# junipertcy/bipartiteSBM-MCMC

Hardware: AMD Instinct MI355X
Metric: node-label MH updates/s (higher is better)
Workload: dtype f64

## Files before the change

### bipartitesbm-mcmc_amd/build.py

```python
import os
import shutil
import subprocess
import sys

HERE = os.path.dirname(os.path.abspath(__file__))
CSRC = os.path.join(HERE, "csrc")
LIB = os.path.join(HERE, "libbisbm_hip.so")
SOURCES = ["bisbm_kernels.hip", "bisbm_sweep_fast.hip", "bisbm_handle.hip", "bisbm_anneal.hip", "bisbm_marginals.hip",
           "bisbm_multi.hip", "bisbm_merge.hip", "bisbm_align.hip", "bisbm_tempering.hip", "bisbm_population.hip", "bisbm_pair_scores.hip", "bisbm_partition.hip",
           "bisbm_query_scores.hip", "bisbm_coassign.hip", "bisbm_foldin.hip", "bisbm_topk.hip", "bisbm_conditionals.hip", "bisbm_heatbath.hip", "bisbm_reshuffle.hip",
           "bisbm_mode_marginals.hip", "bisbm_trace.hip", "bisbm_block_sums.hip", "bisbm_clamp.hip",
           "bisbm_tables.cpp", "bisbm_io.cpp"]
HEADERS = ["bisbm_device.hpp", "bisbm_partition_device.hpp", "bisbm_kernels.hpp", "bisbm_stand_rule.hpp", "bisbm_move_word.hpp", "bisbm_predict_skew.hpp", "bisbm_engine.hpp", "bisbm_pass_policy.hpp", "bisbm_wave_chain.hpp", "bisbm_cand_lanes.hpp", os.path.join("..", "host", "bisbm.hpp"),
           os.path.join("..", "host", "mcmc_main.cpp"), os.path.join("..", "..", "include", "bisbm.h"),
           os.path.join("..", "..", "include", "bisbm_io.h")]
FLAGS = ["--offload-arch=gfx950", "-O3", "-std=c++17", "-ffp-contract=off", "-fPIC", "-pthread",
         "-Wall", "-Wno-unused-function",
         "-mllvm", "-structurizecfg-skip-uniform-regions=true",
         "-mllvm", "-amdgpu-atomic-optimizer-strategy=None",
         "-falign-loops=64"]


def hipcc():
    for cand in (shutil.which("hipcc"), "/opt/rocm/bin/hipcc"):
        if cand and os.path.exists(cand):
            return cand
    raise RuntimeError("hipcc not found: the engine is HIP-only and cannot be built without ROCm")


def needs_build():
    if not os.path.exists(LIB):
        return True
    t = os.path.getmtime(LIB)
    deps = [os.path.join(CSRC, s) for s in SOURCES + HEADERS] + [os.path.abspath(__file__)]
    return any(os.path.getmtime(d) > t for d in deps)


def build(force=False, verbose=False):
    import fcntl
    if not force and not needs_build():
        return LIB
    with open(os.path.join(HERE, ".build.lock"), "w") as lock:
        fcntl.flock(lock, fcntl.LOCK_EX)
        try:
            if not force and not needs_build():
                return LIB
            return _build_locked(verbose)
        finally:
            fcntl.flock(lock, fcntl.LOCK_UN)


RESOURCES = os.path.join(HERE, "libbisbm_hip.resources.json")


def _resource_usage(remarks):
    import re
    out, cur = {}, None
    for line in remarks.splitlines():
        m = re.search(r"remark:\s+Function Name: (\S+)", line)
        if m:
            cur = out.setdefault(m.group(1), {})
            continue
        m = re.search(r"remark:\s+([A-Za-z][^:]*): (\S+) \[-Rpass-analysis", line)
        if m and cur is not None:
            v = m.group(2)
            cur[m.group(1).strip()] = int(v) if v.isdigit() else v
    return out


def compile_library(out, extra=(), verbose=False, jobs=None):
    import tempfile
    from concurrent.futures import ThreadPoolExecutor
    cc = hipcc()
    objdir = tempfile.mkdtemp(prefix="bisbm_obj_")
    try:
        units = []
        for src in SOURCES:
            if src == "bisbm_sweep_fast.hip" and not any("BISBM_STAMPS" in f or "BISBM_PASS_COUNTS" in f for f in extra):
                units += [(src, ["-DBISBM_FAST_PART=%d" % part], "%s.part%d.o" % (src, part)) for part in range(5)]
            else:
                units.append((src, [], src + ".o"))

        def one(unit):
            src, defs, objname = unit
            obj = os.path.join(objdir, objname)
            cmd = [cc] + FLAGS + ["-Rpass-analysis=kernel-resource-usage"] + list(extra) + defs + ["-c", "-o", obj, os.path.join(CSRC, src)]
            if verbose:
                print(" ".join(cmd), file=sys.stderr)
            r = subprocess.run(cmd, capture_output=True, text=True)
            if r.returncode != 0:
                raise RuntimeError("hipcc failed on %s:\n%s%s" % (src, r.stdout, r.stderr))
            return obj, r.stderr
        with ThreadPoolExecutor(max_workers=jobs or min(len(units), os.cpu_count() or 1)) as pool:
            done = list(pool.map(one, units))
        tmp = out + ".tmp%d" % os.getpid()
        cmd = [cc, "--offload-arch=gfx950", "-shared", "-fPIC", "-pthread", "-o", tmp] + [o for o, _ in done]
# ... 50 lines not shown
```

### bipartitesbm-mcmc_amd/csrc/bisbm_sweep_fast.hip

```cpp
#include "bisbm_kernels.hpp"
#include "bisbm_move_word.hpp"
#include "bisbm_stand_rule.hpp"

#include <algorithm>
#include <cstdio>
#include <type_traits>

namespace bisbm {

#ifdef BISBM_STAMPS
__device__ unsigned long long g_fast_stamps[16];
#define FSTAMP(i)                                                                        \
    do {                                                                                 \
        unsigned long long now_;                                                         \
        __builtin_amdgcn_sched_barrier(0);                                               \
        __asm__ volatile("s_memtime %0\n\ts_waitcnt lgkmcnt(0)" : "=s"(now_)::"memory"); \
        __builtin_amdgcn_sched_barrier(0);                                               \
        st_acc[i] += now_ - st_prev;                                                     \
        st_prev = now_;                                                                  \
    } while (0)
#else
#define FSTAMP(i) \
    do {          \
    } while (0)
#endif
#if defined(BISBM_STAMPS) && BISBM_STAMPS == 2
#define FSTAMP_STEP(i) \
    do {               \
    } while (0)
#else
#define FSTAMP_STEP(i) FSTAMP(i)
#endif

__device__ __forceinline__ void wfence() {
    __builtin_amdgcn_wave_barrier();
    __asm__ volatile("" ::: "memory");
}

__device__ __forceinline__ double tab_at(const double* base, uint32_t idx) {
#if defined(BISBM_ABLATE) && (BISBM_ABLATE & 8)
    return (double)idx * 1e-3 + (double)((size_t)base & 0xff);
#endif
    return *(const double*)((const char*)base + (uint32_t)(idx << 3));
}

struct __attribute__((packed, aligned(4))) Id4 {
    uint32_t x, y, z, w;
};

__device__ __forceinline__ uint32_t sflag(uint32_t x) {
    uint32_t r;
    __asm__("s_min_u32 %0, %1, 1" : "=s"(r) : "s"(x) : "scc");
    return r;
}
__device__ __forceinline__ uint32_t smin(uint32_t x, uint32_t y) {
    uint32_t r;
    __asm__("s_min_u32 %0, %1, %2" : "=s"(r) : "s"(x), "s"(y) : "scc");
    return r;
}

struct LaneSwaps {
    __device__ __forceinline__ void swap16(int a, int b, int& x, int& y) const {
        const auto r = __builtin_amdgcn_permlane16_swap(a, b, false, false);
        x = (int)r[0], y = (int)r[1];
    }
    __device__ __forceinline__ void swap32(int a, int b, int& x, int& y) const {
        const auto r = __builtin_amdgcn_permlane32_swap(a, b, false, false);
        x = (int)r[0], y = (int)r[1];
    }
};


#ifdef BISBM_PASS_COUNTS
constexpr int kPassCounts = 15;
__device__ unsigned long long g_pass_counts[kPassCounts];
#define PCOUNT(i, v) (pc_acc[i] += (v))
#define PASS_COUNTS_PAIR(paired)                                                          \
    do {                                                                                  \
        const uint32_t pm_ = (paired) & chA, colk_ = col & sflag(kAtB) & (set_clash ^ 1u); \
        const uint32_t mv_ = target_moves(margin, kAtB);                                  \
        pc_acc[0] += 1u;                                                                  \
        pc_acc[1] += 1u + stands;                                                         \
        pc_acc[2] += pm_;                                                                 \
        pc_acc[3] += pm_ & set_clash;                                                     \
        pc_acc[4] += pm_ & colk_ & (mv_ ^ 1u);                                            \
        pc_acc[5] += pm_ & colk_ & mv_;                                                   \
        pc_acc[6] += pm_ & colk_ & (margin == kAtB ? 1u : 0u);                            \
        pc_acc[7] += pm_ & colk_ & (margin + 1u == kAtB ? 1u : 0u);                       \
    } while (0)
#else
#define PCOUNT(i, v) \
    do {             \
    } while (0)
#define PASS_COUNTS_PAIR(paired) \
    do {                         \
    } while (0)
#endif

#ifndef BISBM_PREDICT_TARGET
#define BISBM_PREDICT_TARGET 1
#endif
constexpr uint32_t kHistStride = 68;
constexpr uint32_t kHandWords = 9;
constexpr uint32_t kRowCap = 255;

#define BISBM_PIN(name, value) \
    double name = (value);     \
    __asm__ volatile("" : "+v"(name))

struct TargetReads {
    uint32_t s_loc, a_st, e_idx, tail_idx;
    int32_t m_st_raw, m_st;
    int ee, qn, qk;
    double logn, tail_lg, L2, L4;
};
struct TargetReads2 {
    uint32_t s_loc, a_st0, a_st1, e_idx, tail_idx;
    int32_t m_st_raw0, m_st_raw1, m_st0, m_st1;
    int ee, qn, qk;
    double logn, tail_lg, L2_0, L2_1, L4_0, L4_1;
};

struct PairSteps {
    uint32_t r_locA, r_locB, degA, degB, t_locB, s_prdA, s_prdB;
    uint32_t liveA, liveB;
    uint32_t selfA, selfB, warmA, warmB;
    uint32_t prop, pack_v, deg, r_loc, t_loc;
    double u_acc;
    __device__ __forceinline__ uint32_t flags(uint32_t clash) const {
        return (liveA & (selfA ^ 1u)) | ((liveA & selfA & warmA) << 1) | ((liveB & (selfB ^ 1u)) << 2) | ((liveB & selfB & warmB) << 3) |
               (clash << 4);
    }
};

__device__ __forceinline__ uint32_t rows4(unsigned long long b) {
    const unsigned long long x = b >> 15;
    return (uint32_t)(x | (x >> 15) | (x >> 30) | (x >> 45)) & 0xfu;
}
__device__ __forceinline__ void commit_four(uint32_t nst, uint32_t clash_bits, uint32_t mv4, uint32_t& moved, uint32_t& commit) {
    const uint32_t c01 = (clash_bits >> 1) & 1u, c02 = (clash_bits >> 2) & 1u, c03 = (clash_bits >> 3) & 1u;
    const uint32_t c12 = (clash_bits >> 6) & 1u, c13 = (clash_bits >> 7) & 1u, c23 = (clash_bits >> 11) & 1u;
    const uint32_t m0 = mv4 & 1u;
    const uint32_t k1 = sflag(nst - 1u) & ((m0 & c01) ^ 1u);
    const uint32_t m1 = k1 & (mv4 >> 1) & 1u;
    const uint32_t k2 = k1 & (nst > 2u ? 1u : 0u) & ((m0 & c02) ^ 1u) & ((m1 & c12) ^ 1u);
    const uint32_t m2 = k2 & (mv4 >> 2) & 1u;
    const uint32_t k3 = k2 & (nst > 3u ? 1u : 0u) & ((m0 & c03) ^ 1u) & ((m1 & c13) ^ 1u) & ((m2 & c23) ^ 1u);
    const uint32_t m3 = k3 & (mv4 >> 3) & 1u;
    commit = 1u | (k1 << 1) | (k2 << 2) | (k3 << 3);
    moved = m0 | (m1 << 1) | (m2 << 2) | (m3 << 3);
}

template <bool EL, bool CT, bool K32, bool K16, bool K8, bool Q32, bool OS>
__device__ __forceinline__ void sweep_fast_body(const SweepParams& p) {
    extern __shared__ __align__(16) uint32_t lds32[];
    const uint32_t chain = blockIdx.x;
    if (chain >= p.n_chains) return;
    const uint32_t lane = threadIdx.x & 63u;
    if (p.resume != 0u && p.scalars[chain].stopped != 0u) {
        if (threadIdx.x == 0) {
            p.scalars[chain].last_accepted = 0;
            p.scalars[chain].last_sweeps = 0;
        }
        return;
    }
    const uint32_t ka = p.ka, kb = p.kb, K = ka + kb, na = p.na, nb = p.nb;
    const uint32_t D = p.maxdeg + 1, S = kb | 1u;
    constexpr bool kPredictTarget = !K16 && (!Q32 || OS) && (BISBM_PREDICT_TARGET != 0);
    const uint32_t row_cap = p.maxdeg < kRowCap ? p.maxdeg : kRowCap;
    const uint32_t o_mq = 0, o_eta = ka * S;
    const uint32_t eta_w = EL ? D : p.eta_w;
    const uint32_t o_hist8 = o_eta + (EL ? K * D : (ka > kb ? ka : kb) * eta_w);
    const uint32_t o_hand = o_hist8 + 2 * kWave * (kHistStride / 4);
    const uint32_t o_slow = o_hand + 2 * kHandWords * kWave;
    const uint32_t o_flag = o_slow + kWave;
    int32_t* const mq = (int32_t*)(lds32 + o_mq);
    uint32_t* const eta_l = lds32 + o_eta;
    uint32_t* const hist8_base = lds32 + o_hist8;
    uint32_t* const hand_base = lds32 + o_hand;
    int32_t* const slow_hist = (int32_t*)(lds32 + o_slow);
    uint32_t* const stop_flag = lds32 + o_flag;
    unsigned long long* const below1_total = (unsigned long long*)(lds32 + ((o_flag + 4u + 1u) & ~1u));
    const uint32_t wave_in_wg = (uint32_t)__builtin_amdgcn_readfirstlane((int)(threadIdx.x >> 6));
    uint32_t hw_id, xcc_id;
    __asm__ volatile("s_getreg_b32 %0, hwreg(HW_REG_HW_ID)" : "=s"(hw_id));
    __asm__ volatile("s_getreg_b32 %0, hwreg(HW_REG_XCC_ID)" : "=s"(xcc_id));
    uint32_t* const role = lds32 + o_flag + 1;
    uint8_t* const new_lab = (uint8_t*)(lds32 + o_flag + 8);
    int32_t* const mr_pub = (int32_t*)(lds32 + o_flag + 24);
    double* const invT_buf = (double*)(lds32 + o_flag + 88);
    if (lane == 0) role[wave_in_wg] = ((xcc_id & 0xfu) << 10) | ((hw_id >> 6) & 0x3fcu) | ((hw_id >> 4) & 3u);
    __syncthreads();
    if (wave_in_wg == 0 && lane == 0) {
        uint32_t pick = p.simd_claims != nullptr ? 0u : (p.fixed_stepping_wave & 1u);
        if (p.simd_claims != nullptr && atomicAdd(&p.simd_claims[role[0]], 1u) != 0u) {
            if (atomicAdd(&p.simd_claims[role[1]], 1u) == 0u) {
                pick = 1;
                atomicSub(&p.simd_claims[role[0]], 1u);
            } else {
                atomicSub(&p.simd_claims[role[1]], 1u);
            }
        }
        role[2] = pick;
    }
    __syncthreads();
    const bool is_main = (uint32_t)__builtin_amdgcn_readfirstlane((int)role[2]) == wave_in_wg;

    uint8_t* const labels = p.labels + (size_t)chain * p.label_stride;
    int32_t* const m_g = p.m + (size_t)chain * ka * kb;
    int32_t* const mr_g = p.m_r + (size_t)chain * K;
    int32_t* const nr_g = p.n_r + (size_t)chain * K;
    uint32_t* const eta_g = p.eta + (size_t)chain * K * D;
    ChainScalars* const sc = p.scalars + chain;
    const Tables tab{p.lgamma_tab, p.lgamma_size, p.q_tab, p.q_stride, p.log_tab};
    if (lane == 0) {
        sc->hw_id[is_main ? 0 : 1] = hw_id;
        if (is_main) sc->xcc_id = xcc_id;
    }

    if (is_main) {
        for (uint32_t i = lane; i < ka * kb; i += kWave) mq[(i / kb) * S + (i % kb)] = m_g[i];
        if (EL)
            for (uint32_t i = lane; i < K * D; i += kWave) eta_l[i] = eta_g[i];
        if (lane == 0) {
            *stop_flag = 0;
            *below1_total = p.resume != 0u ? sc->stop_below1 : 0ull;
        }
    }
    if (is_main) __builtin_amdgcn_s_setprio(3);
    const uint32_t lb = K8 ? (lane & 7u) : K16 ? (lane & 15u) : K32 ? (lane & 31u) : lane;
    int mrA = lb < ka ? mr_g[lb] : 0, nrA = lb < ka ? nr_g[lb] : 0;
    int mrB = lb < kb ? mr_g[ka + lb] : 0, nrB = lb < kb ? nr_g[ka + lb] : 0;
    __syncthreads();
    uint64_t sweeps_total = sc->sweeps_total;

    const double eps = p.epsilon;
    const double Kd = (double)K;
    const double epsK = eps * Kd;
    const uint32_t chain_gid = chain_gid_of(p, chain);
    const uint32_t n = p.n;
    const uint64_t all_sweeps = p.duration / n;
    const double T_const = (double)p.kw0;
    const bool pair_mode = (uint32_t)__builtin_amdgcn_readfirstlane((K32 && (!CT || T_const > 0.) && p.pair_steps != 0) ? 1 : 0) != 0u;
    const bool pair64_mode = (uint32_t)__builtin_amdgcn_readfirstlane((!K32 && (!CT || T_const > 0.) && p.pair_steps != 0) ? 1 : 0) != 0u;
    const bool quad_mode = (uint32_t)__builtin_amdgcn_readfirstlane((K16 && !K8 && (!CT || T_const > 0.) && p.pair_steps > 1u) ? 1 : 0) != 0u;
    const bool quad32_mode = (uint32_t)__builtin_amdgcn_readfirstlane((Q32 && (!CT || T_const > 0.) && p.pair_steps > 1u) ? 1 : 0) != 0u;
    const bool oct_mode = (uint32_t)__builtin_amdgcn_readfirstlane((K8 && (!CT || T_const > 0.) && p.pair_steps > 2u) ? 1 : 0) != 0u;
    const uint32_t track_min =
        (uint32_t)__builtin_amdgcn_readfirstlane((sweep_fast_tracks_minimum(p.schedule, p.kw0, p.steps_await, p.call_duration) || p.keep_sum != 0u) ? 1 : 0);
    BISBM_PIN(c_l2e, 0x1.71547652b82fep+0);
    double c_tol = 1e-5;
// ... 114 lines not shown
                    beg_l = p.rowptr[v_l];
                    deg_l = p.rowptr[v_l + 1] - beg_l;
                    r_l = labels[v_l];
                    const U4 A = phx_draw(p.seed, chain_gid, PHX_STEP_A, sweeps_total * (uint64_t)n + node_base + vi0 + lane);
                    which_l = (uint32_t)(u53(A.x, A.y) * (double)deg_l);
                    if (which_l >= deg_l) which_l = deg_l ? deg_l - 1 : 0;
                }
                for (uint32_t w = 0; w < kHistStride / 4; ++w) hist8w[lane * (kHistStride / 4) + w] = 0;
                wfence();
                const bool mine = lane < cnt && deg_l <= kRowCap;
#if defined(BISBM_ABLATE) && (BISBM_ABLATE & 64)
                const uint32_t my_deg = 0u;
#else
                const uint32_t my_deg = mine ? deg_l : 0u;
#endif
                const int piv_l = (int)labels[my_deg ? p.col[beg_l + which_l] : node_other0];
                {
                    constexpr int U = 16;
                    const uint32_t row_byte0 = lane * kHistStride;
                    for (uint32_t j0 = 0; j0 < row_cap; j0 += U) {
                        if (__ballot(j0 < my_deg) == 0) break;
                        uint32_t idv[U];
#pragma unroll
                        for (int u = 0; u < U; u += 4) {
                            Id4 v4 = {0u, 0u, 0u, 0u};
                            if (j0 + u < my_deg) v4 = *(const Id4*)(p.col + beg_l + j0 + u);
                            idv[u + 0] = v4.x, idv[u + 1] = v4.y, idv[u + 2] = v4.z, idv[u + 3] = v4.w;
                        }
                        int lab[U];
#pragma unroll
                        for (int u = 0; u < U; ++u) {
#if defined(BISBM_ABLATE) && (BISBM_ABLATE & 256)
                            lab[u] = (int)(oth_base + (idv[u] & 31u) % k_oth);
#else
                            lab[u] = labels[j0 + u < my_deg ? idv[u] : node_other0];
#endif
                        }
#pragma unroll
                        for (int u = 0; u < U; ++u) {
                            const uint32_t byte = row_byte0 + (uint32_t)(lab[u] - (int)oth_base);
                            const uint32_t one = j0 + u < my_deg ? 1u : 0u;
#if defined(BISBM_ABLATE) && (BISBM_ABLATE & 128)
                            if (byte == 0xffffffffu) hist8w[0] = one;
#else
                            atomicAdd(&hist8w[byte >> 2], one << ((byte & 3u) * 8u));
#endif
                        }
                    }
                }
                hand[0 * kWave + lane] = v_l;
                hand[1 * kWave + lane] = beg_l;
                hand[2 * kWave + lane] = deg_l;
                hand[3 * kWave + lane] = r_l;
                hand[4 * kWave + lane] = (uint32_t)piv_l;
                double ud_R = 0., ud_tgt = 0., ud_acc = 0.;
                if (lane < cnt) {
                    const uint64_t gs = sweeps_total * (uint64_t)n + node_base + vi0 + lane;
                    const U4 A = phx_draw(p.seed, chain_gid, PHX_STEP_A, gs);
                    const U4 B = phx_draw(p.seed, chain_gid, PHX_STEP_B, gs);
                    ud_R = u53(A.z, A.w);
                    ud_tgt = u53(B.x, B.y);
                    ud_acc = u53(B.z, B.w);
                }
                const uint32_t tloc_l = ((uint32_t)piv_l - oth_base) & 63u;
                const uint32_t rloc_l = r_l - own_base;
                uint32_t prop_l = draw_target(mr_pub[tloc_l], ud_R, ud_tgt);
                if (k_own == 1u || deg_l == 0u || deg_l > kRowCap || (CT && T_const == 0.)) prop_l |= 0x80000000u;
                if (!EL && deg_l - eta_lo >= eta_w) prop_l |= 0x80000000u;
                hand[5 * kWave + lane] = prop_l;
                uint32_t spred_l = 0u;
                if constexpr (kPredictTarget) {
                    const uint32_t x = prop_l & 0x7fffffffu;
                    uint32_t cum = 0u;
                    for (uint32_t i = 0; i < k_own; ++i) {
                        cum += (uint32_t)mq[mq_at(i, tloc_l)];
                        spred_l += cum <= x ? 1u : 0u;
                    }
                    spred_l = spred_l < k_own ? spred_l : k_own - 1u;
                    const uint32_t skew = (uint32_t)__builtin_amdgcn_readfirstlane((int)p.predict_skew);
                    if (__builtin_expect(skew != 0u, 0)) spred_l = skewed_prediction(spred_l, lane, skew, k_own);
                }
                hand[6 * kWave + lane] = (deg_l & 255u) | ((rloc_l & 63u) << 8) | (tloc_l << 16) | (spred_l << 24);
                *(double*)&hand[7 * kWave + 2 * lane] = ud_acc;
                wfence();
            };

            auto run_steps = [&](uint32_t c) {
                const uint32_t vi0 = c * kWave;
                const uint32_t cnt = (n_own - vi0) < (uint32_t)kWave ? (n_own - vi0) : (uint32_t)kWave;
                const uint8_t* const hist8_cur = (const uint8_t*)(hist8_base + (c & 1u) * kWave * (kHistStride / 4));
                const uint32_t* const hand = hand_base + (c & 1u) * kHandWords * kWave;
                new_lab[lane] = 0xffu;
                const uint32_t pack_l = hand[6 * kWave + lane];
                unsigned long long gen_mask = __builtin_amdgcn_ballot_w64((int32_t)hand[5 * kWave + lane] < 0);
                auto prop_of = [&](uint32_t step) -> uint32_t { return hand[5 * kWave + step]; };
                auto u_acc_of = [&](uint32_t step) -> double { return *(const double*)&hand[7 * kWave + 2 * step]; };
                double T_l = T_const;
                if (!CT) T_l = temperature_tabled(p, sweep_step0 + node_base + vi0 + lane);
                const double invT_l = 1.0 / T_l;
                if (!CT && invT_l == INFINITY) T_l = 0.;
                if (!CT) {
                    invT_buf[lane] = invT_l;
                    wfence();
                }
                auto invT_of = [&](uint32_t step) -> double { return invT_buf[step]; };
                auto T_of_step = [&](uint32_t q) -> double {
                    if (CT) return T_const;
                    const double T = temperature_tabled(p, sweep_step0 + node_base + vi0 + q);
                    return 1.0 / T == INFINITY ? 0. : T;
                };
                const unsigned long long below1_mask =
                    track_min != 0u ? __builtin_amdgcn_ballot_w64(lane < cnt && T_l < 1.) : 0ull;
                const unsigned long long below1_before = track_min != 0u ? *below1_total : 0ull;
                auto new_minimum = [&](uint32_t q) {
                    const unsigned long long before =
                        below1_before + (unsigned long long)__builtin_popcountll(below1_mask & ((1ull << q) - 1ull));
                    const bool better = cum_l0 < emin_l0;
                    emin_l0 = better ? cum_l0 : emin_l0;
                    mark_l0 = better ? before : mark_l0;
                };
                auto book = [&](bool ok, double T) {
                    if (ok && lane == 0) acc_l0 += 1;
                };

                auto step_general = [&](uint32_t q, double T) {
                    auto handed = [&](uint32_t word) { return (uint32_t)__builtin_amdgcn_readfirstlane((int)hand[word * kWave + q]); };
                    const uint32_t deg = handed(2), r = handed(3);
                    const uint32_t r_loc = r - own_base;
                    const uint64_t gs_q = sweeps_total * (uint64_t)n + node_base + vi0 + q;
                    const U4 gA = phx_draw(p.seed, chain_gid, PHX_STEP_A, gs_q), gB = phx_draw(p.seed, chain_gid, PHX_STEP_B, gs_q);
                    const double u_idx = u53(gA.x, gA.y), u_R = u53(gA.z, gA.w), u_tgt = u53(gB.x, gB.y), u_acc = u53(gB.z, gB.w);
                    const uint32_t kbyte = q * kHistStride + lane;
                    int k = (int)((((const uint32_t*)hist8_cur)[kbyte >> 2] >> ((kbyte & 3u) * 8u)) & 0xffu);
                    const uint32_t a_rt = mq_at(r_loc, lane);
                    const int32_t m_rt_raw = mq[a_rt];
                    const int32_t m_rt = lane < k_oth ? m_rt_raw : 0;
                    const int eta_r = (int)eta_any_rd(r_loc, deg);
                    uint32_t t_piv = handed(4);
                    if (deg > kRowCap) {
                        const uint32_t beg = handed(1);
                        uint32_t which = (uint32_t)(u_idx * (double)deg);
                        if (which >= deg) which = deg - 1;
                        slow_hist[lane] = 0;
                        wfence();
                        for (uint32_t j = lane; j < deg; j += kWave)
                            atomicAdd(&slow_hist[(int)labels[p.col[beg + j]] - (int)oth_base], 1);
                        wfence();
                        k = lane < k_oth ? slow_hist[lane] : 0;
                        t_piv = labels[p.col[beg + which]];
                    }
                    const int w_piv = mq[mq_at(lane, t_piv - oth_base)];

                    uint32_t s;
                    if (k_own == 1) {
                        s = r;
                    } else if (deg == 0) {
                        s = (uint32_t)(u_idx * Kd);
                        if (s >= K) s = K - 1;
                    } else {
                        const uint32_t prop = draw_target(readlane(mr_oth, t_piv - oth_base), u_R, u_tgt);
                        if ((int32_t)prop < 0) {
                            s = prop & 0x7fffffffu;
                        } else {
                            const int scan = wave_inclusive_scan(w_piv);
                            const unsigned long long hit = __ballot(lane < k_own && (uint32_t)scan > prop);
                            s = hit ? own_base + (uint32_t)__ffsll((long long)hit) - 1 : own_base + k_own - 1;
// ... 656 lines not shown
                    const double a0 = k0 * (t.m_st0 + eps) * inv_lo + k1 * (t.m_st1 + eps) * inv_hi;
                    const double a1 = k0 * (m_rt0 - k0 + eps) * inv_lo + k1 * (m_rt1 - k1 + eps) * inv_hi;
                    double accu0, accu1;
                    butterfly_accu_rows32(a0, a1, accu0, accu1);
                    const double lq = hot_log_q(std::false_type{}, t.qn, t.qk, t.logn);
                    double d = (L1_0 + t.L2_0) - (L3_0 + t.L4_0);
                    d = d + t.tail_lg * sign_tail;
                    d = d + lq * sign_q;
                    d = d + ((L1_1 + t.L2_1) - (L3_1 + t.L4_1));
                    const double dS = butterfly_rows32(d);
                    const unsigned long long b_acc = accept_halves(dS, accu0, accu1, P.u_acc, qs, P.warmA, P.warmB);
                    return pair_commit(
                        tm, q, qB, qs, pair_ok, flags, b_acc, dS, dlA, dlB, dmA, dmB, t.e_idx, t.ee + ((int)(lh & 1u) * 2 - 1), t.s_loc,
                        [&](unsigned long long movers) {
                            if (__builtin_amdgcn_inverse_ballot_w64(movers & lanes_koth64_lo)) {
                                mq[a_rt0] = m_rt_raw0 - k0;
                                mq[t.a_st0] = t.m_st_raw0 + k0;
                            }
                            if (__builtin_amdgcn_inverse_ballot_w64(movers & lanes_koth64_hi)) {
                                mq[a_rt1] = m_rt_raw1 - k1;
                                mq[t.a_st1] = t.m_st_raw1 + k1;
                            }
                        },
                        [&](uint32_t chA, uint32_t stands) { PASS_COUNTS_PAIR(pair_ok); });
                };

                const uint32_t row = lane >> 4;
                constexpr unsigned long long kRowRep = 0x8000800080008000ull;
                auto step_quad = [&](auto tm, uint32_t q, uint32_t nst) -> uint32_t {
                    constexpr bool TM = decltype(tm)::value;
                    const uint32_t qs = q + min(row, nst - 1u);
                    const int sel = (int)(qs << 2);
                    const uint32_t prop = prop_of(qs);
                    const uint32_t pack = (uint32_t)__builtin_amdgcn_ds_bpermute(sel, (int)pack_l);
                    const double u_acc = u_acc_of(qs);
                    const uint32_t deg = pack & 255u, r_loc = (pack >> 8) & 63u, t_loc = (pack >> 16) & 63u;
                    const int k = (int)hist8_cur[qs * kHistStride + lb];
                    const uint32_t a_rt = mq_at(r_loc, lb);
                    const int32_t m_rt_raw = mq[a_rt];
                    const int w_piv = mq[mq_at(lb, t_loc)];
                    const int nn_r = __builtin_amdgcn_ds_bpermute((int)(r_loc << 2), nr_own);
                    const int32_t kmask = (0 - k) >> 31;
                    const int32_t m_rt = m_rt_raw & kmask;
                    const uint32_t kk = (uint32_t)k;
                    const double L1 = tab_at(tab.lg, (uint32_t)(m_rt + 1));
                    const double L3 = tab_at(tab.lg, (uint32_t)(m_rt + 1) - kk);
                    __asm__ volatile("" ::: "memory");
                    const int scan = row_inclusive_scan16(w_piv);
                    const unsigned long long hit = __builtin_amdgcn_ballot_w64((uint32_t)scan > prop);
                    const uint32_t field = (uint32_t)(hit >> (row << 4)) & 0xffffu;
                    const uint32_t s_loc = min((uint32_t)__builtin_ctz(field | 0x10000u), last_own);
                    const unsigned long long m_valid = nst >= 4u ? ~0ull : ((1ull << (16u * nst)) - 1ull);
                    const unsigned long long m_live = __builtin_amdgcn_ballot_w64(nn_r != 1);
                    const unsigned long long m_self = __builtin_amdgcn_ballot_w64(s_loc == r_loc);
                    const unsigned long long m_warm = CT ? ~0ull : ~__builtin_amdgcn_ballot_w64(((zeroT_mask >> qs) & 1ull) != 0ull);
                    const unsigned long long b_can = m_valid & m_live & ~m_self & kRowRep;
                    const unsigned long long b_selfok = m_valid & m_live & m_self & m_warm & kRowRep;
                    if (b_can == 0ull) {
                        acc_chunk += (uint32_t)__builtin_popcountll(b_selfok);
                        if constexpr (TM)
                            if (b_selfok != 0ull) new_minimum(q + ((uint32_t)__builtin_ctzll(b_selfok) >> 4));
                        return nst;
                    }
                    TargetReads t;
                    target_lds(t, s_loc, r_loc, deg, kmask);
                    target_gathers(t, kk, std::false_type{});
                    const double a0 = k * (t.m_st + eps) * inv_blk;
                    const double a1 = k * (m_rt - k + eps) * inv_blk;
                    const double accu0 = butterfly_rows16(a0);
                    const double accu1 = butterfly_rows16(a1);
                    const double lq = hot_log_q(std::true_type{}, t.qn, t.qk, t.logn);
                    const uint32_t clash_bits =
                        (uint32_t)clash_pairs(Four{}, r_loc, s_loc, t_loc, pack_margins(margin_up((uint32_t)scan, (uint32_t)w_piv, prop), margin_down((uint32_t)scan, prop)),
                                              (int)(((lane >> 2) & 3u) << 6), (int)((lane & 3u) << 6), [&](int li, uint32_t t_j) {
                            return (uint32_t)__builtin_amdgcn_ds_bpermute(li + (int)(t_j << 2), (int)kk);
                        }) & 0xffffu;
                    double d = (L1 + t.L2) - (L3 + t.L4);
                    d = d + t.tail_lg * sign_tail;
                    d = d + lq * sign_q;
                    const double dS = butterfly_rows16(d);
                    const unsigned long long b_acc = accept_rows(dS, accu0, accu1, u_acc, qs, m_warm, b_can);
                    const uint32_t mv4 = rows4(b_can & b_acc), selfok4 = rows4(b_selfok);
                    uint32_t moved, commit;
                    commit_four(nst, clash_bits, mv4, moved, commit);
#ifdef BISBM_PASS_COUNTS
                    count_pairs((lane >> 2) & 3u, lane & 3u, lane < 16u, moved, commit, nst);
#endif
                    apply_moves(tm, Four{}, q, qs, row, moved, commit & selfok4, r_loc, s_loc, deg, std::false_type{}, 0, 0, dS, t.e_idx, t.ee, [&](unsigned long long movers) {
                        if (__builtin_amdgcn_inverse_ballot_w64(movers & lanes_koth)) {
                            mq[a_rt] = m_rt_raw - k;
                            mq[t.a_st] = t.m_st_raw + k;
                        }
                    });
                    return (uint32_t)__builtin_popcount(commit);
                };
                auto step_quad32 = [&](auto tm, uint32_t q, uint32_t nst) -> uint32_t {
                    constexpr bool TM = decltype(tm)::value;
                    const uint32_t qs = q + min(row, nst - 1u);
                    const int sel = (int)(qs << 2);
                    const uint32_t prop = prop_of(qs);
                    const uint32_t pack = (uint32_t)__builtin_amdgcn_ds_bpermute(sel, (int)pack_l);
                    const double u_acc = u_acc_of(qs);
                    const uint32_t deg = pack & 255u, r_loc = (pack >> 8) & 63u, t_loc = (pack >> 16) & 63u;
                    const int k0 = (int)hist8_cur[qs * kHistStride + l16], k1 = (int)hist8_cur[qs * kHistStride + l16 + 16u];
                    const uint32_t a_rt0 = mq_at(r_loc, l16), a_rt1 = mq_at(r_loc, l16 + 16u);
                    const int32_t m_rt_raw0 = mq[a_rt0], m_rt_raw1 = mq[a_rt1];
                    const int w0 = mq[mq_at(l16, t_loc)], w1 = mq[mq_at(l16 + 16u, t_loc)];
                    const int nn_r = __builtin_amdgcn_ds_bpermute((int)(r_loc << 2), nr_own);
                    const int32_t kmask0 = (0 - k0) >> 31, kmask1 = (0 - k1) >> 31;
                    const int32_t m_rt0 = m_rt_raw0 & kmask0, m_rt1 = m_rt_raw1 & kmask1;
                    const uint32_t kk0 = (uint32_t)k0, kk1 = (uint32_t)k1;
                    const double L1_0 = tab_at(tab.lg, (uint32_t)(m_rt0 + 1)), L3_0 = tab_at(tab.lg, (uint32_t)(m_rt0 + 1) - kk0);
                    const double L1_1 = tab_at(tab.lg, (uint32_t)(m_rt1 + 1)), L3_1 = tab_at(tab.lg, (uint32_t)(m_rt1 + 1) - kk1);
                    TargetReads2 t;
                    if constexpr (OS && kPredictTarget) {
                        target_lds2(t, pack >> 24, r_loc, deg, kmask0, kmask1, l16, 16u);
                        target_gathers2(t, kk0, kk1, std::true_type{});
                    }
                    __asm__ volatile("" ::: "memory");
                    const int scan0 = row_inclusive_scan16(w0);
                    int tot = w0;
                    tot += __builtin_amdgcn_update_dpp(0, tot, kDppXor1, 0xF, 0xF, false);
                    tot += __builtin_amdgcn_update_dpp(0, tot, kDppXor2, 0xF, 0xF, false);
                    tot += __builtin_amdgcn_update_dpp(0, tot, kDppHalfMirror, 0xF, 0xF, false);
                    tot += __builtin_amdgcn_update_dpp(0, tot, kDppMirror, 0xF, 0xF, false);
                    const int scan1 = row_inclusive_scan16(w1) + tot;
                    const unsigned long long hit0 = __builtin_amdgcn_ballot_w64((uint32_t)scan0 > prop);
                    const unsigned long long hit1 = __builtin_amdgcn_ballot_w64((uint32_t)scan1 > prop);
                    const uint32_t field = ((uint32_t)(hit0 >> (row << 4)) & 0xffffu) | ((uint32_t)(hit1 >> (row << 4)) << 16);
                    const uint32_t s_loc = min((uint32_t)__builtin_ctz(field | 0x80000000u), last_own);
                    if constexpr (OS && kPredictTarget) {
                        const unsigned long long wrong =
                            __builtin_amdgcn_ballot_w64(s_loc != (pack >> 24)) & kRowRep & (nst >= 4u ? ~0ull : ((1ull << (16u * nst)) - 1ull));
                        uint32_t first_wrong;
                        __asm__("s_ff1_i32_b64 %0, %1" : "=s"(first_wrong) : "s"(wrong));
                        const uint32_t nst_ok = smin(nst, first_wrong >> 4);
                        PCOUNT(13, nst_ok == 0u ? 1u : 0u);
                        PCOUNT(14, (nst_ok != 0u && nst_ok < nst) ? 1u : 0u);
                        if (__builtin_expect(nst_ok == 0u, 0)) return 0u;
                        nst = nst_ok;
                    }
                    const unsigned long long m_valid = nst >= 4u ? ~0ull : ((1ull << (16u * nst)) - 1ull);
                    const unsigned long long m_live = __builtin_amdgcn_ballot_w64(nn_r != 1);
                    const unsigned long long m_self = __builtin_amdgcn_ballot_w64(s_loc == r_loc);
                    const unsigned long long m_warm = CT ? ~0ull : ~__builtin_amdgcn_ballot_w64(((zeroT_mask >> qs) & 1ull) != 0ull);
                    const unsigned long long b_can = m_valid & m_live & ~m_self & kRowRep;
                    const unsigned long long b_selfok = m_valid & m_live & m_self & m_warm & kRowRep;
                    if (b_can == 0ull) {
                        acc_chunk += (uint32_t)__builtin_popcountll(b_selfok);
                        if constexpr (TM)
                            if (b_selfok != 0ull) new_minimum(q + ((uint32_t)__builtin_ctzll(b_selfok) >> 4));
                        return nst;
                    }
                    if constexpr (!(OS && kPredictTarget)) {
                        target_lds2(t, s_loc, r_loc, deg, kmask0, kmask1, l16, 16u);
                        target_gathers2(t, kk0, kk1, std::true_type{});
                    }
                    const uint32_t leaf_m = 0u - (s_loc >> 4);
                    const uint32_t S_own = (uint32_t)scan0 ^ (((uint32_t)scan0 ^ (uint32_t)scan1) & leaf_m);
                    const uint32_t w_own = (uint32_t)w0 ^ (((uint32_t)w0 ^ (uint32_t)w1) & leaf_m);
                    uint32_t margins = pack_margins(margin_up(S_own, w_own, prop), margin_down(S_own, prop));
                    __asm__ volatile("" : "+v"(margins));
                    const double a0 = k0 * (t.m_st0 + eps) * invq_lo + k1 * (t.m_st1 + eps) * invq_hi;
                    const double a1 = k0 * (m_rt0 - k0 + eps) * invq_lo + k1 * (m_rt1 - k1 + eps) * invq_hi;
                    const double accu0 = butterfly_rows16(a0);
                    const double accu1 = butterfly_rows16(a1);
                    const double lq = hot_log_q(std::false_type{}, t.qn, t.qk, t.logn);
                    const uint32_t clash_bits =
                        (uint32_t)clash_pairs(Four{}, r_loc, s_loc, t_loc, margins,
                                              (int)(((lane >> 2) & 3u) << 6), (int)((lane & 3u) << 6), [&](int li, uint32_t t_j) {
                            const int src = li + (int)((t_j & 15u) << 2);
                            const uint32_t k_lo = (uint32_t)__builtin_amdgcn_ds_bpermute(src, (int)kk0);
                            const uint32_t k_hi = (uint32_t)__builtin_amdgcn_ds_bpermute(src, (int)kk1);
                            return k_lo ^ ((k_lo ^ k_hi) & (0u - (t_j >> 4)));
                        }) & 0xffffu;
                    int zw_lo = 0, zw_hi = 0;
                    if constexpr (OS) {
                        zw_lo = move_word(r_loc, s_loc, deg, l16), zw_hi = move_word(r_loc, s_loc, deg, l16 + 16u);
                        __asm__ volatile("" : "+v"(zw_lo), "+v"(zw_hi));
                    }
                    double d0 = (L1_0 + t.L2_0) - (L3_0 + t.L4_0);
                    d0 = d0 + t.tail_lg * sign_tail;
                    d0 = d0 + lq * sign_q;
                    const double d1 = (L1_1 + t.L2_1) - (L3_1 + t.L4_1);
                    const double dS = butterfly_rows16(d1) + butterfly_rows16(d0);
                    const unsigned long long b_acc = accept_rows(dS, accu0, accu1, u_acc, qs, m_warm, b_can);
                    const uint32_t mv4 = rows4(b_can & b_acc), selfok4 = rows4(b_selfok);
                    uint32_t moved, commit;
                    commit_four(nst, clash_bits, mv4, moved, commit);
#ifdef BISBM_PASS_COUNTS
                    count_pairs((lane >> 2) & 3u, lane & 3u, lane < 16u, moved, commit, nst);
#endif
                    apply_moves(tm, Four{}, q, qs, row, moved, commit & selfok4, r_loc, s_loc, deg, std::bool_constant<OS>{}, zw_lo, zw_hi, dS, t.e_idx, t.ee, [&](unsigned long long movers) {
                        if (__builtin_amdgcn_inverse_ballot_w64(movers & lanes_koth32_lo)) {
                            mq[a_rt0] = m_rt_raw0 - k0;
                            mq[t.a_st0] = t.m_st_raw0 + k0;
                        }
                        if (__builtin_amdgcn_inverse_ballot_w64(movers & lanes_koth32_hi)) {
                            mq[a_rt1] = m_rt_raw1 - k1;
                            mq[t.a_st1] = t.m_st_raw1 + k1;
                        }
                    });
                    return (uint32_t)__builtin_popcount(commit);
                };
                const uint32_t grp = lane >> 3;
                auto step_oct = [&](auto tm, uint32_t q, uint32_t nst) -> uint32_t {
                    constexpr bool TM = decltype(tm)::value;
                    const uint32_t qs = q + min(grp, nst - 1u);
                    const int sel = (int)(qs << 2);
                    const uint32_t prop = prop_of(qs);
                    const uint32_t pack = (uint32_t)__builtin_amdgcn_ds_bpermute(sel, (int)pack_l);
                    const double u_acc = u_acc_of(qs);
                    const uint32_t deg = pack & 255u, r_loc = (pack >> 8) & 63u, t_loc = (pack >> 16) & 63u;
                    const int k = (int)hist8_cur[qs * kHistStride + lb];
                    const uint32_t a_rt = mq_at(r_loc, lb);
                    const int32_t m_rt_raw = mq[a_rt];
                    const int w_piv = mq[mq_at(lb, t_loc)];
                    const int nn_r = __builtin_amdgcn_ds_bpermute((int)(r_loc << 2), nr_own);
                    const int32_t kmask = (0 - k) >> 31;
                    const int32_t m_rt = m_rt_raw & kmask;
                    const uint32_t kk = (uint32_t)k;
                    const double L1 = tab_at(tab.lg, (uint32_t)(m_rt + 1));
                    const double L3 = tab_at(tab.lg, (uint32_t)(m_rt + 1) - kk);
                    __asm__ volatile("" ::: "memory");
                    const int scan = group_inclusive_scan8(w_piv, lb);
                    const unsigned long long hit = __builtin_amdgcn_ballot_w64((uint32_t)scan > prop);
                    const uint32_t field = (uint32_t)(hit >> (grp << 3)) & 0xffu;
                    const uint32_t s_loc = min((uint32_t)__builtin_ctz(field | 0x100u), last_own);
                    const unsigned long long m_valid = nst >= 8u ? ~0ull : ((1ull << (8u * nst)) - 1ull);
                    const unsigned long long m_live = __builtin_amdgcn_ballot_w64(nn_r != 1);
                    const unsigned long long m_self = __builtin_amdgcn_ballot_w64(s_loc == r_loc);
                    const unsigned long long m_warm = CT ? ~0ull : ~__builtin_amdgcn_ballot_w64(((zeroT_mask >> qs) & 1ull) != 0ull);
                    constexpr unsigned long long kGrpRep = 0x8080808080808080ull;
                    const unsigned long long b_can = m_valid & m_live & ~m_self & kGrpRep;
                    const unsigned long long b_selfok = m_valid & m_live & m_self & m_warm & kGrpRep;
                    if (b_can == 0ull) {
                        acc_chunk += (uint32_t)__builtin_popcountll(b_selfok);
                        if constexpr (TM)
                            if (b_selfok != 0ull) new_minimum(q + ((uint32_t)__builtin_ctzll(b_selfok) >> 3));
                        return nst;
                    }
                    TargetReads t;
                    target_lds(t, s_loc, r_loc, deg, kmask);
                    target_gathers(t, kk, std::false_type{});
                    const double a0 = k * (t.m_st + eps) * inv_blk;
                    const double a1 = k * (m_rt - k + eps) * inv_blk;
                    const double accu0 = butterfly_groups8(a0);
                    const double accu1 = butterfly_groups8(a1);
                    const double lq = hot_log_q(std::true_type{}, t.qn, t.qk, t.logn);
                    const unsigned long long clash_bits =
                        clash_pairs(Eight{}, r_loc, s_loc, t_loc, pack_margins(margin_up((uint32_t)scan, (uint32_t)w_piv, prop), margin_down((uint32_t)scan, prop)),
                                    (int)((lane & 7u) << 5), (int)((lane >> 3) << 5), [&](int li, uint32_t t_j) {
                            return (uint32_t)__builtin_amdgcn_ds_bpermute(li + (int)(t_j << 2), (int)kk);
                        });
                    double d = (L1 + t.L2) - (L3 + t.L4);
                    d = d + t.tail_lg * sign_tail;
                    d = d + lq * sign_q;
                    const double dS = butterfly_groups8(d);
                    const unsigned long long b_acc = accept_rows(dS, accu0, accu1, u_acc, qs, m_warm, b_can);
                    auto groups8 = [](unsigned long long b) -> uint32_t { return (uint32_t)(((b >> 7) * 0x0102040810204080ull) >> 56) & 0xffu; };
                    const uint32_t mv8 = groups8(b_can & b_acc), selfok8 = groups8(b_selfok);
                    uint32_t moved = mv8 & 1u, commit = 1u, stands = 1u;
#pragma unroll
                    for (uint32_t j = 1; j < 8u; ++j) {
                        const uint32_t clash_j = (uint32_t)(clash_bits >> (8u * j)) & moved;
                        stands &= (nst > j ? 1u : 0u) & (clash_j == 0u ? 1u : 0u);
                        commit |= stands << j;
                        moved |= (stands & (mv8 >> j) & 1u) << j;
                    }
#ifdef BISBM_PASS_COUNTS
                    count_pairs(lane & 7u, lane >> 3, true, moved, commit, nst);
#endif
// ... 257 lines not shown
```

Baseline: 2.379 billion.

## Precompute pairwise clash fields in hand-prep to simplify four-step clash detection

Adds a per-lane packed pair word, computed once during hand preparation, that encodes for each of the three preceding lanes the shared/outside block relation and the histogram count toward this lane's target. The four-step deep pass then derives clash bits with one ballot over a table lookup against a permuted margin, replacing the clash_pairs routine and its paired ds_bpermute gathers. commit_four is templated on the bit positions so it can read clash bits in either layout. The cost is extra LDS word storage, extra bpermutes and fences in hand prep, and more code that must match the old clash rule exactly.

```diff
diff --git a/bipartitesbm-mcmc_amd/build.py b/bipartitesbm-mcmc_amd/build.py
--- a/bipartitesbm-mcmc_amd/build.py
+++ b/bipartitesbm-mcmc_amd/build.py
@@ -11,7 +11,7 @@
            "bisbm_query_scores.hip", "bisbm_coassign.hip", "bisbm_foldin.hip", "bisbm_topk.hip", "bisbm_conditionals.hip", "bisbm_heatbath.hip", "bisbm_reshuffle.hip",
            "bisbm_mode_marginals.hip", "bisbm_trace.hip", "bisbm_block_sums.hip", "bisbm_clamp.hip",
            "bisbm_tables.cpp", "bisbm_io.cpp"]
-HEADERS = ["bisbm_device.hpp", "bisbm_partition_device.hpp", "bisbm_kernels.hpp", "bisbm_stand_rule.hpp", "bisbm_move_word.hpp", "bisbm_predict_skew.hpp", "bisbm_engine.hpp", "bisbm_pass_policy.hpp", "bisbm_wave_chain.hpp", "bisbm_cand_lanes.hpp", os.path.join("..", "host", "bisbm.hpp"),
+HEADERS = ["bisbm_device.hpp", "bisbm_partition_device.hpp", "bisbm_kernels.hpp", "bisbm_stand_rule.hpp", "bisbm_pair_word.hpp", "bisbm_move_word.hpp", "bisbm_predict_skew.hpp", "bisbm_engine.hpp", "bisbm_pass_policy.hpp", "bisbm_wave_chain.hpp", "bisbm_cand_lanes.hpp", os.path.join("..", "host", "bisbm.hpp"),
            os.path.join("..", "host", "mcmc_main.cpp"), os.path.join("..", "..", "include", "bisbm.h"),
            os.path.join("..", "..", "include", "bisbm_io.h")]
 FLAGS = ["--offload-arch=gfx950", "-O3", "-std=c++17", "-ffp-contract=off", "-fPIC", "-pthread",
diff --git a/bipartitesbm-mcmc_amd/csrc/bisbm_pair_word.hpp b/bipartitesbm-mcmc_amd/csrc/bisbm_pair_word.hpp
--- /dev/null
+++ b/bipartitesbm-mcmc_amd/csrc/bisbm_pair_word.hpp
@@ -0,0 +1,32 @@
+#pragma once
+
+#include <cstdint>
+
+#include "bisbm_stand_rule.hpp"
+
+namespace bisbm {
+
+constexpr uint32_t kPairFieldBits = 10u;
+constexpr uint32_t kPairMarginsTop = (kMarginCap + 1u) << 16;
+
+BISBM_RULE_FN uint32_t pair_word_field(uint32_t r_i, uint32_t s_i, uint32_t r_j, uint32_t s_j, uint32_t k_i_tj) {
+    const uint32_t common = ((1u << r_i) | (1u << s_i)) & ((1u << r_j) | (1u << s_j));
+    const uint32_t shared = common < 1u ? common : 1u;
+    const uint32_t outside = ((blocks_between(r_i, s_i) >> s_j) & 1u) ^ 1u;
+    const uint32_t down = (r_i - s_i) >> 31;
+    const uint32_t sel = ((shared | outside) << 1) | ((shared ^ 1u) & (down | outside));
+    return (k_i_tj & 0xffu) | (sel << 8);
+}
+
+template <uint32_t D>
+BISBM_RULE_FN uint32_t pair_clash(uint32_t field, uint32_t margins_j) {
+    static_assert(D == 4u || D == 8u, "depth of a deep pass");
+    const uint64_t table = ((uint64_t)kPairMarginsTop << 32) | margins_j;
+    const uint32_t margin = ((uint32_t)(table >> ((field >> 4) & 0x30u)) & 0xffffu) - 1u;
+    return target_moves(margin, (D - 1u) * (field & 0xffu));
+}
+
+BISBM_RULE_FN uint32_t pair_word(uint32_t f1, uint32_t f2, uint32_t f3) { return f1 | (f2 << kPairFieldBits) | (f3 << (2u * kPairFieldBits)); }
+BISBM_RULE_FN uint32_t pair_word_at(uint32_t word, uint32_t d) { return (word >> (kPairFieldBits * (d - 1u))) & ((1u << kPairFieldBits) - 1u); }
+
+}
diff --git a/bipartitesbm-mcmc_amd/csrc/bisbm_sweep_fast.hip b/bipartitesbm-mcmc_amd/csrc/bisbm_sweep_fast.hip
--- a/bipartitesbm-mcmc_amd/csrc/bisbm_sweep_fast.hip
+++ b/bipartitesbm-mcmc_amd/csrc/bisbm_sweep_fast.hip
@@ -1,5 +1,6 @@
 #include "bisbm_kernels.hpp"
 #include "bisbm_move_word.hpp"
+#include "bisbm_pair_word.hpp"
 #include "bisbm_stand_rule.hpp"
 
 #include <algorithm>
@@ -101,7 +102,7 @@
 #define BISBM_PREDICT_TARGET 1
 #endif
 constexpr uint32_t kHistStride = 68;
-constexpr uint32_t kHandWords = 9;
+constexpr uint32_t kHandWords = 10;
 constexpr uint32_t kRowCap = 255;
 
 #define BISBM_PIN(name, value) \
@@ -137,9 +138,16 @@
     const unsigned long long x = b >> 15;
     return (uint32_t)(x | (x >> 15) | (x >> 30) | (x >> 45)) & 0xfu;
 }
-__device__ __forceinline__ void commit_four(uint32_t nst, uint32_t clash_bits, uint32_t mv4, uint32_t& moved, uint32_t& commit) {
-    const uint32_t c01 = (clash_bits >> 1) & 1u, c02 = (clash_bits >> 2) & 1u, c03 = (clash_bits >> 3) & 1u;
-    const uint32_t c12 = (clash_bits >> 6) & 1u, c13 = (clash_bits >> 7) & 1u, c23 = (clash_bits >> 11) & 1u;
+struct PairsByLane4 {
+    static constexpr uint32_t p01 = 1, p02 = 2, p03 = 3, p12 = 6, p13 = 7, p23 = 11;
+};
+struct PairsByRow {
+    static constexpr uint32_t p01 = 16, p02 = 33, p03 = 50, p12 = 32, p13 = 49, p23 = 48;
+};
+template <class At, class Bits>
+__device__ __forceinline__ void commit_four(At, uint32_t nst, Bits clash_bits, uint32_t mv4, uint32_t& moved, uint32_t& commit) {
+    const uint32_t c01 = (uint32_t)(clash_bits >> At::p01) & 1u, c02 = (uint32_t)(clash_bits >> At::p02) & 1u, c03 = (uint32_t)(clash_bits >> At::p03) & 1u;
+    const uint32_t c12 = (uint32_t)(clash_bits >> At::p12) & 1u, c13 = (uint32_t)(clash_bits >> At::p13) & 1u, c23 = (uint32_t)(clash_bits >> At::p23) & 1u;
     const uint32_t m0 = mv4 & 1u;
     const uint32_t k1 = sflag(nst - 1u) & ((m0 & c01) ^ 1u);
     const uint32_t m1 = k1 & (mv4 >> 1) & 1u;
@@ -167,6 +175,11 @@
     const uint32_t ka = p.ka, kb = p.kb, K = ka + kb, na = p.na, nb = p.nb;
     const uint32_t D = p.maxdeg + 1, S = kb | 1u;
     constexpr bool kPredictTarget = !K16 && (!Q32 || OS) && (BISBM_PREDICT_TARGET != 0);
+#ifdef BISBM_PASS_COUNTS
+    constexpr bool kPairWord = false;
+#else
+    constexpr bool kPairWord = kPredictTarget && Q32 && OS;
+#endif
     const uint32_t row_cap = p.maxdeg < kRowCap ? p.maxdeg : kRowCap;
     const uint32_t o_mq = 0, o_eta = ka * S;
     const uint32_t eta_w = EL ? D : p.eta_w;
@@ -447,6 +460,21 @@
                 }
                 hand[6 * kWave + lane] = (deg_l & 255u) | ((rloc_l & 63u) << 8) | (tloc_l << 16) | (spred_l << 24);
                 *(double*)&hand[7 * kWave + 2 * lane] = ud_acc;
+                if constexpr (kPairWord) {
+                    wfence();
+                    const uint32_t rs_l = (rloc_l & 31u) | ((spred_l & 31u) << 8);
+                    uint32_t lane_o = lane;
+                    __asm__ volatile("" : "+v"(lane_o));
+                    uint32_t f[3];
+#pragma unroll
+                    for (uint32_t d = 1; d <= 3u; ++d) {
+                        const uint32_t src = (lane_o - d) & 63u;
+                        const uint32_t rs_i = (uint32_t)__builtin_amdgcn_ds_bpermute((int)(src << 2), (int)rs_l);
+                        const uint32_t k_i_tj = ((const uint8_t*)hist8w)[src * kHistStride + tloc_l];
+                        f[d - 1u] = pair_word_field(rs_i & 31u, rs_i >> 8, rloc_l & 31u, spred_l & 31u, k_i_tj);
+                    }
+                    hand[9 * kWave + lane] = pair_word(f[0], f[1], f[2]);
+                }
                 wfence();
             };
 
@@ -1269,7 +1297,7 @@
                     const unsigned long long b_acc = accept_rows(dS, accu0, accu1, u_acc, qs, m_warm, b_can);
                     const uint32_t mv4 = rows4(b_can & b_acc), selfok4 = rows4(b_selfok);
                     uint32_t moved, commit;
-                    commit_four(nst, clash_bits, mv4, moved, commit);
+                    commit_four(PairsByLane4{}, nst, clash_bits, mv4, moved, commit);
 #ifdef BISBM_PASS_COUNTS
                     count_pairs((lane >> 2) & 3u, lane & 3u, lane < 16u, moved, commit, nst);
 #endif
@@ -1353,14 +1381,22 @@
                     const double accu0 = butterfly_rows16(a0);
                     const double accu1 = butterfly_rows16(a1);
                     const double lq = hot_log_q(std::false_type{}, t.qn, t.qk, t.logn);
-                    const uint32_t clash_bits =
-                        (uint32_t)clash_pairs(Four{}, r_loc, s_loc, t_loc, margins,
-                                              (int)(((lane >> 2) & 3u) << 6), (int)((lane & 3u) << 6), [&](int li, uint32_t t_j) {
+                    unsigned long long clash_bits;
+                    if constexpr (kPairWord) {
+                        uint32_t m_c = margins;
+                        __asm__ volatile("" : "+v"(m_c)::"memory");
+                        const uint32_t pairs = hand[9 * kWave + qs];
+                        const uint32_t margins_j = (uint32_t)__builtin_amdgcn_ds_bpermute((int)(((lane & 48u) | (s_loc & 15u)) << 2), (int)m_c);
+                        clash_bits = __builtin_amdgcn_ballot_w64(pair_clash<4u>(pairs >> ((kPairFieldBits * l16) & 31u), margins_j) != 0u);
+                    } else {
+                        clash_bits = clash_pairs(Four{}, r_loc, s_loc, t_loc, margins,
+                                                 (int)(((lane >> 2) & 3u) << 6), (int)((lane & 3u) << 6), [&](int li, uint32_t t_j) {
                             const int src = li + (int)((t_j & 15u) << 2);
                             const uint32_t k_lo = (uint32_t)__builtin_amdgcn_ds_bpermute(src, (int)kk0);
                             const uint32_t k_hi = (uint32_t)__builtin_amdgcn_ds_bpermute(src, (int)kk1);
                             return k_lo ^ ((k_lo ^ k_hi) & (0u - (t_j >> 4)));
-                        }) & 0xffffu;
+                        }) & 0xffffull;
+                    }
                     int zw_lo = 0, zw_hi = 0;
                     if constexpr (OS) {
                         zw_lo = move_word(r_loc, s_loc, deg, l16), zw_hi = move_word(r_loc, s_loc, deg, l16 + 16u);
@@ -1374,7 +1410,10 @@
                     const unsigned long long b_acc = accept_rows(dS, accu0, accu1, u_acc, qs, m_warm, b_can);
                     const uint32_t mv4 = rows4(b_can & b_acc), selfok4 = rows4(b_selfok);
                     uint32_t moved, commit;
-                    commit_four(nst, clash_bits, mv4, moved, commit);
+                    if constexpr (kPairWord)
+                        commit_four(PairsByRow{}, nst, clash_bits, mv4, moved, commit);
+                    else
+                        commit_four(PairsByLane4{}, nst, (uint32_t)clash_bits, mv4, moved, commit);
 #ifdef BISBM_PASS_COUNTS
                     count_pairs((lane >> 2) & 3u, lane & 3u, lane < 16u, moved, commit, nst);
 #endif
```

New measurement: 2.459 billion (median of 6 runs). +3.4%, better.
